# 0215Arthur/Pytorch_News_Recommender

Measured on AMD Instinct MI355X. Metric: users/sec (train step) NRMS MIND-small hist=50 cand=5, higher is better.
Workload: dtype f16 (MFMA inputs and saved activations; fp32 accumulate, softmax, loss, master weights and Adam); 1 GPU; configs[1] shapes: NRMS(nrms_v0) train step, 512 users/GPU, hist=50, cand=5, title_len=30, d=300, h=10, q=200, V=45800, dropout=0.2, Adam(lr=1e-3); users_per_gpu=512, global_batch=512, parallelism=dp1, precision=fp16, resident_batches=32

## Files before the change

### pytorch_news_recommender_amd/csrc/embed.hip

```cpp
#include "gemm.h"

#include <algorithm>

namespace nrms {

__global__ __launch_bounds__(256) void gather_dropout_kernel(unsigned total4, unsigned d4, const int64_t* ids,
                                                             const float* table, Dropout drop, float* x) {
    const unsigned stride = gridDim.x * blockDim.x;
    for (unsigned i = blockIdx.x * blockDim.x + threadIdx.x; i < total4; i += stride) {
        const unsigned m = i / d4, c4 = i - m * d4;
        const long id = ids[m];
        f32x4 v = *reinterpret_cast<const f32x4*>(table + id * (long)(4 * d4) + 4 * c4);
        if (drop.thresh != 0u) v *= dropout_scale4(drop.seed, 0u, (uint64_t)i, drop.thresh, drop.inv_keep);
        reinterpret_cast<f32x4*>(x)[i] = v;
    }
}

__global__ __launch_bounds__(256) void gather_dropout_compact_kernel(unsigned d4, const int64_t* ids, const int* live,
                                                                     const int* n_live, const float* table, Dropout drop,
                                                                     float* x) {
    const unsigned total4 = (unsigned)(*n_live) * d4;
    const unsigned stride = gridDim.x * blockDim.x;
    for (unsigned i = blockIdx.x * blockDim.x + threadIdx.x; i < total4; i += stride) {
        const unsigned r = i / d4, c4 = i - r * d4;
        const long t = live[r];
        f32x4 v = *reinterpret_cast<const f32x4*>(table + ids[t] * (long)(4 * d4) + 4 * c4);
        if (drop.thresh != 0u) v *= dropout_scale4(drop.seed, 0u, (uint64_t)(t * d4 + c4), drop.thresh, drop.inv_keep);
        reinterpret_cast<f32x4*>(x)[i] = v;
    }
}

int launch_gather_dropout_compact(long M, int d, const int64_t* ids, const int* live, const int* n_live,
                                  const float* table, const Dropout& drop, float* x, hipStream_t stream) {
    if (M <= 0) return NRMS_OK;
    if (M * (d / 4) >= (1L << 32)) { set_error("gather: %ld float4 elements overflow the 32-bit index", M * (d / 4)); return NRMS_EINVAL; }
    int blocks = cdiv(M * (d / 4), 256);
    if (blocks > 256 * 16) blocks = 256 * 16;
    TimingScope ts("gather_dropout", stream);
    hipLaunchKernelGGL(gather_dropout_compact_kernel, dim3(blocks), dim3(256), 0, stream, (unsigned)(d / 4), ids, live,
                       n_live, table, drop, x);
    return check_launch("gather_dropout");
}

template <bool SKIP_ALL_PAD, int FILL_SLICES>
__global__ __launch_bounds__(256) void fill_pad_rows_kernel_t(long n_seq, int S, int n4, const int64_t* ids, const float* row,
                                                              float* out) {
    const int lane = threadIdx.x & 63;
    const long wave = (long)blockIdx.x * 4 + (threadIdx.x >> 6), n_waves = (long)gridDim.x * 4;
    f32x4 b[FILL_SLICES];
#pragma unroll
    for (int i = 0; i < FILL_SLICES; ++i)
        b[i] = (lane + 64 * i < n4) ? reinterpret_cast<const f32x4*>(row)[lane + 64 * i] : f32x4{0.f, 0.f, 0.f, 0.f};
    for (long q = wave; q < n_seq; q += n_waves) {
        const bool is_pad = lane < S && ids[q * S + lane] == 0;
        unsigned long long m = __ballot(is_pad);
        if (SKIP_ALL_PAD && __popcll(m) == S) continue;
        while (m != 0ull) {
            const int r = __builtin_ctzll(m);
            m &= m - 1ull;
            f32x4* o = reinterpret_cast<f32x4*>(out) + (q * S + r) * n4;
#pragma unroll
            for (int i = 0; i < FILL_SLICES; ++i)
                if (lane + 64 * i < n4) o[lane + 64 * i] = b[i];
        }
    }
}

int launch_fill_pad_rows(long n_seq, int S, int n, const int64_t* ids, const float* row, float* out, bool skip_all_pad,
                         hipStream_t stream) {
    if (n_seq <= 0) return NRMS_OK;
    if ((n & 3) != 0 || n > 256 * 12 || S > 64) { set_error("fill_pad_rows: n=%d S=%d unsupported", n, S); return NRMS_EINVAL; }
    int blocks = cdiv(n_seq, 4);
    if (blocks > 256 * 32) blocks = 256 * 32;
    TimingScope ts("fill_pad_rows", stream);
    const bool wide = n > 256 * 6;
    auto go = [&](auto kernel) { hipLaunchKernelGGL(kernel, dim3(blocks), dim3(256), 0, stream, n_seq, S, n / 4, ids, row, out); };
    if (skip_all_pad) { if (wide) go(fill_pad_rows_kernel_t<true, 12>); else go(fill_pad_rows_kernel_t<true, 6>); }
    else { if (wide) go(fill_pad_rows_kernel_t<false, 12>); else go(fill_pad_rows_kernel_t<false, 6>); }
    return check_launch("fill_pad_rows");
}

constexpr int CP_BLOCK = 1024;
__global__ __launch_bounds__(256) void compact_count_kernel(long M, const int64_t* ids, int* counts) {
    __shared__ int wsum[4];
    const long m0 = (long)blockIdx.x * CP_BLOCK;
    int c = 0;
#pragma unroll
    for (int p = 0; p < 4; ++p) {
        const long m = m0 + p * 256 + threadIdx.x;
        c += (m < M && ids[m] != 0) ? 1 : 0;
    }
    c = (int)wave_sum((float)c);
    if ((threadIdx.x & 63) == 0) wsum[threadIdx.x >> 6] = c;
    __syncthreads();
    if (threadIdx.x == 0) counts[blockIdx.x] = wsum[0] + wsum[1] + wsum[2] + wsum[3];
}

__global__ __launch_bounds__(1024) void compact_scan_kernel(int n_blocks, int* counts, int* n_live) {
    __shared__ int buf[1024];
    __shared__ int carry;
    if (threadIdx.x == 0) carry = 0;
    __syncthreads();
    for (int base = 0; base < n_blocks; base += 1024) {
        const int i = base + threadIdx.x;
        const int v = i < n_blocks ? counts[i] : 0;
        buf[threadIdx.x] = v;
        __syncthreads();
        for (int off = 1; off < 1024; off <<= 1) {
            const int t = threadIdx.x >= off ? buf[threadIdx.x - off] : 0;
            __syncthreads();
            buf[threadIdx.x] += t;
            __syncthreads();
        }
        if (i < n_blocks) counts[i] = carry + buf[threadIdx.x] - v;
        __syncthreads();
        if (threadIdx.x == 1023) carry += buf[1023];
        __syncthreads();
    }
    if (threadIdx.x == 0) *n_live = carry;
}

__global__ __launch_bounds__(256) void compact_write_kernel(long M, const int64_t* ids, const int* offsets, int* live,
                                                            int* pos) {
    __shared__ int wave_cnt[4][4];
    const int lane = threadIdx.x & 63, wave = threadIdx.x >> 6;
    const long m0 = (long)blockIdx.x * CP_BLOCK;
    bool flag[4];
    int pre[4];
#pragma unroll
    for (int p = 0; p < 4; ++p) {
        const long m = m0 + p * 256 + threadIdx.x;
        flag[p] = m < M && ids[m] != 0;
        const unsigned long long b = __ballot(flag[p]);
        pre[p] = __popcll(b & ((1ull << lane) - 1ull));
        if (lane == 0) wave_cnt[p][wave] = __popcll(b);
    }
    __syncthreads();
    if (threadIdx.x == 0) {
        int tot = 0;
        for (int p = 0; p < 4; ++p)
            for (int w = 0; w < 4; ++w) { const int c = wave_cnt[p][w]; wave_cnt[p][w] = tot; tot += c; }
    }
    __syncthreads();
    const int base = offsets[blockIdx.x];
#pragma unroll
    for (int p = 0; p < 4; ++p) {
        const long m = m0 + p * 256 + threadIdx.x;
        const int r = base + wave_cnt[p][wave] + pre[p];
        if (flag[p]) live[r] = (int)m;
        if (pos != nullptr && m < M) pos[m] = flag[p] ? r : -1;
    }
}

size_t compact_scratch_ints(long M) { return (size_t)cdiv(M, CP_BLOCK) + 64; }

int launch_compact_live_rows(long M, const int64_t* ids, int* live, int* pos, int* n_live, int* scratch,
                             hipStream_t stream) {
    if (M <= 0) return NRMS_OK;
    const int nb = cdiv(M, CP_BLOCK);
    TimingScope ts("compact_rows", stream);
    hipLaunchKernelGGL(compact_count_kernel, dim3(nb), dim3(256), 0, stream, M, ids, scratch);
    hipLaunchKernelGGL(compact_scan_kernel, dim3(1), dim3(1024), 0, stream, nb, scratch, n_live);
    hipLaunchKernelGGL(compact_write_kernel, dim3(nb), dim3(256), 0, stream, M, ids, scratch, live, pos);
    return check_launch("compact_live_rows");
}

template <typename IDX>
__global__ __launch_bounds__(256) void scatter_dropout_compact_kernel(unsigned d, const int64_t* ids, const int* live,
                                                                      const int* n_live, const float* dx, Dropout drop,
                                                                      float* dtable) {
    const IDX total = (IDX)(*n_live) * d;
    const IDX stride = (IDX)gridDim.x * blockDim.x;
    for (IDX i = (IDX)blockIdx.x * blockDim.x + threadIdx.x; i < total; i += stride) {
        const IDX r = i / d;
        const unsigned c = (unsigned)(i - r * d);
        const long t = live[r];
        const long id = ids[t];
        float v = dx[i];
        if (drop.thresh != 0u) v *= dropout_scale1(drop.seed, 0u, (uint64_t)(t * d + c), drop.thresh, drop.inv_keep);
        atomicAdd(dtable + id * (long)d + c, v);
    }
}

__global__ __launch_bounds__(256) void scatter_dense_rows_kernel(unsigned d, const int64_t* ids, const int* live,
                                                                 const int* n_live, const float* dx, Dropout drop, float* dtable) {
    const unsigned long total = (unsigned long)(*n_live) * d;
    const unsigned long stride = (unsigned long)gridDim.x * blockDim.x;
    for (unsigned long i = (unsigned long)blockIdx.x * blockDim.x + threadIdx.x; i < total; i += stride) {
        const unsigned long r = i / d;
        const unsigned c = (unsigned)(i - r * d);
        const long t = live[r];
        float v = dx[t * (long)d + c];
        if (drop.thresh != 0u) v *= dropout_scale1(drop.seed, 0u, (uint64_t)(t * d + c), drop.thresh, drop.inv_keep);
        atomicAdd(dtable + ids[t] * (long)d + c, v);
    }
}

int launch_scatter_dense_rows(long M, int d, const int64_t* ids, const int* live, const int* n_live, const float* dx,
                              const Dropout& drop, float* dtable, hipStream_t stream) {
    if (M <= 0) return NRMS_OK;
    int blocks = cdiv(M * d, 256);
    if (blocks > 256 * 16) blocks = 256 * 16;
    TimingScope ts("scatter_dropout", stream);
    hipLaunchKernelGGL(scatter_dense_rows_kernel, dim3(blocks), dim3(256), 0, stream, (unsigned)d, ids, live, n_live, dx, drop, dtable);
    return check_launch("scatter_dense_rows");
}

int launch_scatter_dropout_compact(long M, int d, const int64_t* ids, const int* live, const int* n_live, const float* dx,
                                   const Dropout& drop, float* dtable, hipStream_t stream) {
    if (M <= 0) return NRMS_OK;
    int blocks = cdiv(M * d, 256);
    if (blocks > 256 * 16) blocks = 256 * 16;
    TimingScope ts("scatter_dropout", stream);
    if (M * d < (1L << 32))
        hipLaunchKernelGGL(scatter_dropout_compact_kernel<unsigned>, dim3(blocks), dim3(256), 0, stream, (unsigned)d, ids,
                           live, n_live, dx, drop, dtable);
    else
        hipLaunchKernelGGL(scatter_dropout_compact_kernel<unsigned long>, dim3(blocks), dim3(256), 0, stream, (unsigned)d, ids,
                           live, n_live, dx, drop, dtable);
    return check_launch("scatter_dropout");
}

__global__ __launch_bounds__(256) void tok_hist_kernel(const int64_t* ids, const int* live, const int* n_live, int* cnt) {
    const int n = *n_live;
    for (int r = blockIdx.x * blockDim.x + threadIdx.x; r < n; r += gridDim.x * blockDim.x)
        atomicAdd(cnt + ids[live[r]], 1);
}

__global__ __launch_bounds__(1024) void scan_local_kernel(int n, int* data, int* bsum) {
    __shared__ int buf[1024];
    const int i = blockIdx.x * 1024 + threadIdx.x;
    const int v = i < n ? data[i] : 0;
    buf[threadIdx.x] = v;
    __syncthreads();
    for (int off = 1; off < 1024; off <<= 1) {
        const int t = threadIdx.x >= off ? buf[threadIdx.x - off] : 0;
        __syncthreads();
        buf[threadIdx.x] += t;
        __syncthreads();
    }
    if (i < n) data[i] = buf[threadIdx.x] - v;
    if (threadIdx.x == 1023) bsum[blockIdx.x] = buf[1023];
}

__global__ __launch_bounds__(1024) void scan_add_kernel(int n, int n_blocks, int* data, const int* bsum, int* total) {
    __shared__ int base;
    if (threadIdx.x == 0) {
        int s = 0;
        for (int b = 0; b < (int)blockIdx.x; ++b) s += bsum[b];
        base = s;
        if (blockIdx.x == n_blocks - 1) *total = s + bsum[blockIdx.x];
    }
    __syncthreads();
    const int i = blockIdx.x * 1024 + threadIdx.x;
    if (i < n) data[i] += base;
}

__global__ __launch_bounds__(256) void tok_place_kernel(const int64_t* ids, const int* live, const int* n_live,
                                                        const int* offs, int* cursor, int* order) {
    const int n = *n_live;
    for (int r = blockIdx.x * blockDim.x + threadIdx.x; r < n; r += gridDim.x * blockDim.x) {
        const long id = ids[live[r]];
        order[offs[id] + atomicAdd(cursor + id, 1)] = r;
    }
}

typedef _Float16 sg_h4 __attribute__((ext_vector_type(4)));
template <bool H16, int SL>
__device__ __forceinline__ void bucket_sum(f32x4 (&s)[SL], int lane, int d4, int beg, int end, const int* live, const int* order,
                                           const void* dxv, int ldx, const Dropout& drop) {
    const float* dx = reinterpret_cast<const float*>(dxv);
    const _Float16* dx16 = reinterpret_cast<const _Float16*>(dxv);
    auto add_row = [&](int r) {
        const long t = live[r];
#pragma unroll
        for (int j = 0; j < SL; ++j) {
            const int c4 = lane + 64 * j;
            if (c4 < d4) {
                f32x4 g;
                if (H16) {
                    const sg_h4 gh = *reinterpret_cast<const sg_h4*>(dx16 + (long)r * ldx + 4 * c4);
#pragma unroll
                    for (int e = 0; e < 4; ++e) g[e] = (float)gh[e];
                } else {
                    g = *reinterpret_cast<const f32x4*>(dx + ((long)r * d4 + c4) * 4);
                }
                if (drop.thresh != 0u) g *= dropout_scale4(drop.seed, 0u, (uint64_t)(t * d4 + c4), drop.thresh, drop.inv_keep);
                s[j] += g;
            }
        }
    };
    constexpr int NONE = 0x7fffffff;
    for (int k0 = beg; k0 < end; k0 += 256) {
        const int n = min(256, end - k0);
        int m0 = lane < n ? order[k0 + lane] : NONE, m1 = lane + 64 < n ? order[k0 + 64 + lane] : NONE;
        int m2 = lane + 128 < n ? order[k0 + 128 + lane] : NONE, m3 = lane + 192 < n ? order[k0 + 192 + lane] : NONE;
        for (int i = 0; i < n; ++i) {
            int m = min(min(m0, m1), min(m2, m3));
#pragma unroll
            for (int o = 32; o > 0; o >>= 1) m = min(m, __shfl_xor(m, o, 64));
            add_row(m);
            m0 = m0 == m ? NONE : m0;
            m1 = m1 == m ? NONE : m1;
            m2 = m2 == m ? NONE : m2;
            m3 = m3 == m ? NONE : m3;
        }
    }
}

template <bool H16, int SL = 2>
__global__ __launch_bounds__(256) void scatter_grouped_kernel(int V, int d4, const int* live, const int* offs,
                                                              const int* total, const int* order, const void* dxv, int ldx,
                                                              const float* sc, Dropout drop, float* dtable) {
    const int lane = threadIdx.x & 63;
    const int v = blockIdx.x * 4 + (threadIdx.x >> 6);
    if (v >= V || v == 0) return;
    const int beg = offs[v], end = v + 1 < V ? offs[v + 1] : *total;
    if (beg == end) return;
    f32x4 s[SL];
#pragma unroll
    for (int j = 0; j < SL; ++j) s[j] = f32x4{0.f, 0.f, 0.f, 0.f};
    bucket_sum<H16, SL>(s, lane, d4, beg, end, live, order, dxv, ldx, drop);
#pragma unroll
    for (int j = 0; j < SL; ++j) {
        const int c4 = lane + 64 * j;
        if (c4 < d4) *reinterpret_cast<f32x4*>(dtable + ((long)v * d4 + c4) * 4) += H16 ? s[j] * sc[1] : s[j];
    }
}

template <bool H16, int SL, bool GUARD>
__global__ __launch_bounds__(256) void scatter_grouped_adam_kernel(int V, int d4, const int* live, const int* offs,
                                                                   const int* total, const int* order, const void* dxv, int ldx,
                                                                   const float* sc, Dropout drop, float* dtable, TableAdam a) {
    const int lane = threadIdx.x & 63;
    const int v = blockIdx.x * 4 + (threadIdx.x >> 6);
    if (v >= V) return;
    f32x4 s[SL];
#pragma unroll
    for (int j = 0; j < SL; ++j) s[j] = f32x4{0.f, 0.f, 0.f, 0.f};
    if (v != 0) {
        const int beg = offs[v], end = v + 1 < V ? offs[v + 1] : *total;
        bucket_sum<H16, SL>(s, lane, d4, beg, end, live, order, dxv, ldx, drop);
    }
    const long row4 = (long)v * d4;
    int bad = 0;
#pragma unroll
    for (int j = 0; j < SL; ++j) {
        const int c4 = lane + 64 * j;
        if (c4 < d4) {
            f32x4 g = f32x4{0.f, 0.f, 0.f, 0.f};
            g += H16 ? s[j] * sc[1] : s[j];
            f32x4 pv = reinterpret_cast<const f32x4*>(a.p)[row4 + c4];
            f32x4 mv = reinterpret_cast<const f32x4*>(a.m)[row4 + c4];
            f32x4 vv = reinterpret_cast<const f32x4*>(a.v)[row4 + c4];
            reinterpret_cast<f32x4*>(dtable)[row4 + c4] = g;
            const f32x4 gv = g * a.gscale;
#pragma unroll
            for (int e = 0; e < 4; ++e) {
                const bool skip = GUARD && (__float_as_uint(gv[e]) & 0x7F800000u) == 0x7F800000u;
                float pe = pv[e], me = mv[e], ve = vv[e];
                adam_update(pe, me, ve, gv[e], a.c.step_size, a.c.b1, a.c.b2, a.c.omb1, a.c.omb2, a.c.inv_sqrt_bc2, a.c.eps);
                pv[e] = skip ? pv[e] : pe; mv[e] = skip ? mv[e] : me; vv[e] = skip ? vv[e] : ve;
                bad += skip ? 1 : 0;
            }
            reinterpret_cast<f32x4*>(a.p)[row4 + c4] = pv;
            reinterpret_cast<f32x4*>(a.m)[row4 + c4] = mv;
            reinterpret_cast<f32x4*>(a.v)[row4 + c4] = vv;
        }
    }
    if (GUARD) {
#pragma unroll
        for (int o = 32; o > 0; o >>= 1) bad += __shfl_xor(bad, o, 64);
        if (bad != 0 && lane == 0) atomicAdd(a.n_bad, bad);
    }
}

static size_t scan_blocks(int V) { return (size_t)cdiv(V, 1024); }
size_t scatter_grouped_scratch_ints(long M, int V) { return (size_t)2 * (V + 64) + std::max((size_t)M, scan_blocks(V)) + 64; }

int launch_scatter_prepare(long M, int V, const int64_t* ids, const int* live, const int* n_live, int* scratch, hipStream_t stream) {
    if (M <= 0) return NRMS_OK;
    int* cnt = scratch;
    int* cursor = cnt + V + 64;
    int* total = cursor + V;
    int* order = cursor + V + 64;
    if (hipMemsetAsync(cnt, 0, (size_t)(2 * (V + 64)) * sizeof(int), stream) != hipSuccess) {
        set_error("scatter_grouped: memset failed");
        return NRMS_ELAUNCH;
    }
    int blocks = cdiv(M, 256);
    if (blocks > 2048) blocks = 2048;
    TimingScope ts("scatter_prepare", stream);
    hipLaunchKernelGGL(tok_hist_kernel, dim3(blocks), dim3(256), 0, stream, ids, live, n_live, cnt);
    {
        const int nb = (int)scan_blocks(V);
        int* bsum = order;
        hipLaunchKernelGGL(scan_local_kernel, dim3(nb), dim3(1024), 0, stream, V, cnt, bsum);
        hipLaunchKernelGGL(scan_add_kernel, dim3(nb), dim3(1024), 0, stream, V, nb, cnt, bsum, total);
    }
    hipLaunchKernelGGL(tok_place_kernel, dim3(blocks), dim3(256), 0, stream, ids, live, n_live, cnt, cursor, order);
    return check_launch("scatter_prepare");
}

int launch_scatter_grouped(long M, int V, int d, const int64_t* ids, const int* live, const int* n_live, const void* dx,
                           const Dropout& drop, float* dtable, int* scratch, hipStream_t stream, bool dx_fp16, int ldx,
                           const float* sc, bool prepared) {
    if (M <= 0) return NRMS_OK;
    if ((d & 3) != 0 || d > 1024 || (dx_fp16 && d > 512)) { set_error("scatter_grouped: d=%d unsupported", d); return NRMS_EINVAL; }
    if (!prepared) {
        const int rc = launch_scatter_prepare(M, V, ids, live, n_live, scratch, stream);
        if (rc) return rc;
    }
    int* cnt = scratch;
    int* cursor = cnt + V + 64;
    int* total = cursor + V;
    int* order = cursor + V + 64;
    TimingScope ts("scatter_dropout", stream);
    if (dx_fp16)
        hipLaunchKernelGGL(scatter_grouped_kernel<true>, dim3(cdiv(V, 4)), dim3(256), 0, stream, V, d / 4, live, cnt, total, order, dx,
                           ldx, sc, drop, dtable);
    else if (d <= 512)
        hipLaunchKernelGGL(scatter_grouped_kernel<false>, dim3(cdiv(V, 4)), dim3(256), 0, stream, V, d / 4, live, cnt, total, order, dx,
                           d, nullptr, drop, dtable);
    else
        hipLaunchKernelGGL((scatter_grouped_kernel<false, 4>), dim3(cdiv(V, 4)), dim3(256), 0, stream, V, d / 4, live, cnt, total, order,
                           dx, d, nullptr, drop, dtable);
    return check_launch("scatter_grouped");
}

int launch_scatter_grouped_adam(long M, int V, int d, const int64_t* ids, const int* live, const int* n_live, const void* dx,
                                const Dropout& drop, float* dtable, int* scratch, hipStream_t stream, bool dx_fp16, int ldx,
                                const float* sc, bool prepared, const TableAdam& a) {
    if (M <= 0 || V <= 0) { set_error("scatter_grouped_adam: nothing to scatter (the caller runs the plain Adam step)"); return NRMS_EINVAL; }
    if ((d & 3) != 0 || d > 1024 || (dx_fp16 && d > 512)) { set_error("scatter_grouped_adam: d=%d unsupported", d); return NRMS_EINVAL; }
    if (!prepared) {
        const int rc = launch_scatter_prepare(M, V, ids, live, n_live, scratch, stream);
        if (rc) return rc;
    }
    int* cnt = scratch;
    int* cursor = cnt + V + 64;
    int* total = cursor + V;
    int* order = cursor + V + 64;
    const bool guard = a.n_bad != nullptr;
    TimingScope ts("adam", stream);
    auto go = [&](auto kernel, int ld, const float* scp) {
        hipLaunchKernelGGL(kernel, dim3(cdiv(V, 4)), dim3(256), 0, stream, V, d / 4, live, cnt, total, order, dx, ld, scp, drop, dtable, a);
    };
    if (dx_fp16) { if (guard) go(scatter_grouped_adam_kernel<true, 2, true>, ldx, sc); else go(scatter_grouped_adam_kernel<true, 2, false>, ldx, sc); }
    else if (d <= 512) { if (guard) go(scatter_grouped_adam_kernel<false, 2, true>, d, nullptr); else go(scatter_grouped_adam_kernel<false, 2, false>, d, nullptr); }
    else { if (guard) go(scatter_grouped_adam_kernel<false, 4, true>, d, nullptr); else go(scatter_grouped_adam_kernel<false, 4, false>, d, nullptr); }
    return check_launch("scatter_grouped_adam");
}

template <class SRC>
__global__ __launch_bounds__(256) void sanitize_ids_kernel(long n, const SRC* src, int64_t* dst, long vocab, int* n_bad) {
    int bad = 0;
    for (long i = (long)blockIdx.x * blockDim.x + threadIdx.x; i < n; i += (long)gridDim.x * blockDim.x) {
        const int64_t v = (int64_t)src[i];
        const bool ok = v >= 0 && v < vocab;
        bad += ok ? 0 : 1;
        dst[i] = ok ? v : 0;
    }
    const unsigned long long m = __ballot(bad != 0);
    if (m != 0ull) {
        bad = (int)wave_sum((float)bad);
        if ((threadIdx.x & 63) == 0) atomicAdd(n_bad, bad);
    }
}

int launch_sanitize_ids(long n, const void* src, bool src_is_int32, int64_t* dst, int vocab, int* n_bad, hipStream_t stream) {
    if (n <= 0) return NRMS_OK;
    int blocks = cdiv(n, 256 * 4);
    if (blocks > 256 * 8) blocks = 256 * 8;
    TimingScope ts("sanitize_ids", stream);
    if (src_is_int32)
        hipLaunchKernelGGL(sanitize_ids_kernel<int32_t>, dim3(blocks), dim3(256), 0, stream, n, (const int32_t*)src, dst, (long)vocab, n_bad);
    else
        hipLaunchKernelGGL(sanitize_ids_kernel<int64_t>, dim3(blocks), dim3(256), 0, stream, n, (const int64_t*)src, dst, (long)vocab, n_bad);
    return check_launch("sanitize_ids");
}

__global__ __launch_bounds__(256) void dedup_insert_kernel(long n, int L, const int64_t* ids, int* table, unsigned mask,
                                                           int* inverse, int* rep_rows, int* n_unique) {
    const int lane = threadIdx.x & 63;
    for (long t = (long)blockIdx.x * blockDim.x + threadIdx.x; t < n; t += (long)gridDim.x * blockDim.x) {
        const int64_t* row = ids + t * L;
        uint64_t h = 0x9E3779B97F4A7C15ull ^ (uint64_t)L;
        int64_t any = 0;
        for (int i = 0; i < L; ++i) {
            const int64_t w = row[i];
            any |= w;
            uint64_t k = (uint64_t)w * 0xFF51AFD7ED558CCDull;
            k ^= k >> 32;
            h = (h ^ k) * 0xC4CEB9FE1A85EC53ull;
            h ^= h >> 29;
        }
        h ^= h >> 33; h *= 0xFF51AFD7ED558CCDull; h ^= h >> 33;
        const bool pad = any == 0;
        const unsigned long long pads = __ballot(pad);
        const int leader = pads != 0 ? __ffsll((long long)pads) - 1 : 0;
        int result = 0;
        if (!pad || lane == leader) {
            unsigned slot = (unsigned)h & mask;
            for (;;) {
                int cur = __hip_atomic_load(table + slot, __ATOMIC_RELAXED, __HIP_MEMORY_SCOPE_AGENT);
                if (cur < 0) {
                    cur = atomicCAS(table + slot, -1, (int)t);
                    if (cur < 0) {
                        const int u = atomicAdd(n_unique, 1);
                        rep_rows[u] = (int)t;
                        result = u;
                        break;
                    }
                }
                const int64_t* other = ids + (long)cur * L;
                bool same = true;
                for (int i = 0; i < L; ++i) same = same && other[i] == row[i];
                if (same) { result = -cur - 1; break; }
                slot = (slot + 1) & mask;
            }
        }
        const int lead = __shfl(result, leader);
        inverse[t] = (pad && lane != leader) ? lead : result;
    }
}

__global__ __launch_bounds__(256) void dedup_resolve_kernel(long n, int* inverse) {
    for (long t = (long)blockIdx.x * blockDim.x + threadIdx.x; t < n; t += (long)gridDim.x * blockDim.x) {
        const int v = inverse[t];
        if (v < 0) inverse[t] = inverse[-v - 1];
    }
}

int launch_title_dedup(long n, int L, const int64_t* ids, int* table, long table_size, int* inverse, int* rep_rows,
                       int* n_unique, hipStream_t stream) {
    if (hipMemsetAsync(n_unique, 0, sizeof(int), stream) != hipSuccess) { set_error("title_dedup: memset failed"); return NRMS_ELAUNCH; }
    if (n <= 0) return NRMS_OK;
    if (hipMemsetAsync(table, 0xFF, (size_t)table_size * sizeof(int), stream) != hipSuccess) {
        set_error("title_dedup: memset failed");
        return NRMS_ELAUNCH;
    }
    int blocks = cdiv(n, 256);
    if (blocks > 256 * 16) blocks = 256 * 16;
    TimingScope ts("title_dedup", stream);
    hipLaunchKernelGGL(dedup_insert_kernel, dim3(blocks), dim3(256), 0, stream, n, L, ids, table, (unsigned)(table_size - 1),
                       inverse, rep_rows, n_unique);
    hipLaunchKernelGGL(dedup_resolve_kernel, dim3(blocks), dim3(256), 0, stream, n, inverse);
    return check_launch("title_dedup");
}

int launch_gather_dropout(long M, int d, const int64_t* ids, const float* table, const Dropout& drop, float* x,
                          hipStream_t stream) {
    if (M <= 0) return NRMS_OK;
    const long total4 = M * (d / 4);
    if (total4 >= (1L << 32)) { set_error("gather: %ld float4 elements overflow the 32-bit index", total4); return NRMS_EINVAL; }
    int blocks = cdiv(total4, 256);
    if (blocks > 256 * 16) blocks = 256 * 16;
    TimingScope ts("gather_dropout", stream);
    hipLaunchKernelGGL(gather_dropout_kernel, dim3(blocks), dim3(256), 0, stream, (unsigned)total4, (unsigned)(d / 4),
                       ids, table, drop, x);
    return check_launch("gather_dropout");
}

}
```

Before: 180,500 users/s.

## Rank-sort bucket rows once and prefetch rows ahead in grouped embedding scatter

Replaces the per-row wave-wide min-reduction in the grouped embedding-gradient scatter with a one-time rank computation. Each bucket's row indices are ordered by readlane comparisons and a permute, then walked with a software-pipelined loop that loads upcoming rows a fixed lookahead ahead of the accumulation. This is meant to remove the serial shuffle reduction per row and to hide gather latency. The change uses more registers for the prefetched rows and adds code complexity. The old min-select path stays available behind an environment variable and remains the only path for SL=4.

Result: no change. 182,000 users/s, median of 6 (+0.8%).

```diff
diff --git a/pytorch_news_recommender_amd/csrc/embed.hip b/pytorch_news_recommender_amd/csrc/embed.hip
--- a/pytorch_news_recommender_amd/csrc/embed.hip
+++ b/pytorch_news_recommender_amd/csrc/embed.hip
@@ -1,6 +1,8 @@
 #include "gemm.h"
 
 #include <algorithm>
+#include <stdlib.h>
+#include <type_traits>
 
 namespace nrms {
 
@@ -266,11 +268,12 @@
 }
 
 typedef _Float16 sg_h4 __attribute__((ext_vector_type(4)));
-template <bool H16, int SL>
+template <bool H16, int SL, bool MINSEL, int LA>
 __device__ __forceinline__ void bucket_sum(f32x4 (&s)[SL], int lane, int d4, int beg, int end, const int* live, const int* order,
                                            const void* dxv, int ldx, const Dropout& drop) {
     const float* dx = reinterpret_cast<const float*>(dxv);
     const _Float16* dx16 = reinterpret_cast<const _Float16*>(dxv);
+    typedef typename std::conditional<H16, sg_h4, f32x4>::type row_t;
     auto add_row = [&](int r) {
         const long t = live[r];
 #pragma unroll
@@ -290,9 +293,31 @@
             }
         }
     };
+    auto load_row_all = [&](row_t (&q)[SL], int r) {
+#pragma unroll
+        for (int j = 0; j < SL; ++j) {
+            const int c4 = min(lane + 64 * j, d4 - 1);
+            if constexpr (H16) q[j] = *reinterpret_cast<const sg_h4*>(dx16 + (long)r * ldx + 4 * c4);
+            else q[j] = *reinterpret_cast<const f32x4*>(dx + ((long)r * d4 + c4) * 4);
+        }
+    };
+    auto add_row_all = [&](const row_t (&q)[SL], long t) {
+#pragma unroll
+        for (int j = 0; j < SL; ++j) {
+            const int c4 = lane + 64 * j;
+            f32x4 g;
+            if constexpr (H16) {
+#pragma unroll
+                for (int e = 0; e < 4; ++e) g[e] = (float)q[j][e];
+            } else {
+                g = q[j];
+            }
+            if (drop.thresh != 0u) g *= dropout_scale4(drop.seed, 0u, (uint64_t)(t * d4 + c4), drop.thresh, drop.inv_keep);
+            s[j] += g;
+        }
+    };
     constexpr int NONE = 0x7fffffff;
-    for (int k0 = beg; k0 < end; k0 += 256) {
-        const int n = min(256, end - k0);
+    auto minsel_chunk = [&](int k0, int n) {
         int m0 = lane < n ? order[k0 + lane] : NONE, m1 = lane + 64 < n ? order[k0 + 64 + lane] : NONE;
         int m2 = lane + 128 < n ? order[k0 + 128 + lane] : NONE, m3 = lane + 192 < n ? order[k0 + 192 + lane] : NONE;
         for (int i = 0; i < n; ++i) {
@@ -305,10 +330,87 @@
             m2 = m2 == m ? NONE : m2;
             m3 = m3 == m ? NONE : m3;
         }
-    }
-}
-
-template <bool H16, int SL = 2>
+    };
+    if constexpr (MINSEL || SL == 4) {
+        for (int k0 = beg; k0 < end; k0 += 256) minsel_chunk(k0, min(256, end - k0));
+        return;
+    }
+    constexpr int LA_SHORT = LA, LA_LONG = 0;
+    auto walk = [&](auto la, int n, auto entry) {
+        constexpr int A = decltype(la)::value, R = A + 1;
+        row_t q[R][SL];
+        int r, t;
+        if (n <= A) {
+#pragma unroll
+            for (int a = 0; a < A; ++a)
+                if (a < n) { entry(a, r, t); load_row_all(q[a], r); }
+#pragma unroll
+            for (int a = 0; a < A; ++a)
+                if (a < n) { entry(a, r, t); add_row_all(q[a], (long)t); }
+            return;
+        }
+#pragma unroll
+        for (int a = 0; a < A; ++a) { entry(a, r, t); load_row_all(q[a], r); }
+        for (int i = 0;;) {
+#pragma unroll
+            for (int u = 0; u < R; ++u) {
+                entry(min(i + A, n - 1), r, t);
+                load_row_all(q[(u + A) % R], r);
+                entry(i, r, t);
+                add_row_all(q[u], (long)t);
+                if (++i == n) return;
+            }
+        }
+    };
+    const int kbeg = __builtin_amdgcn_readfirstlane(beg), kend = __builtin_amdgcn_readfirstlane(end);
+    for (int k0 = kbeg; k0 < kend; k0 += 256) {
+        const int n = min(256, kend - k0);
+        if (n <= 64) {
+            int m0 = lane < n ? order[k0 + lane] : NONE;
+            int t0 = lane < n ? live[m0] : 0;
+            if (n > 1) {
+                int rk = 0;
+                for (int j = 0; j < n; ++j) rk += __builtin_amdgcn_readlane(m0, j) < m0 ? 1 : 0;
+                rk = lane < n ? rk : lane;
+                m0 = __builtin_amdgcn_ds_permute(rk << 2, m0);
+                t0 = __builtin_amdgcn_ds_permute(rk << 2, t0);
+            }
+            walk(std::integral_constant<int, LA_SHORT>{}, n, [&](int i, int& r, int& t) {
+                r = __builtin_amdgcn_readlane(m0, i);
+                t = __builtin_amdgcn_readlane(t0, i);
+            });
+        } else {
+            int m[4], t4[4], rk[4];
+#pragma unroll
+            for (int q = 0; q < 4; ++q) {
+                m[q] = lane + 64 * q < n ? order[k0 + 64 * q + lane] : NONE;
+                rk[q] = 0;
+            }
+#pragma unroll
+            for (int q = 0; q < 4; ++q) t4[q] = lane + 64 * q < n ? live[m[q]] : 0;
+#pragma unroll
+            for (int q = 0; q < 4; ++q) {
+                const int cnt = min(64, n - 64 * q);
+                for (int j = 0; j < cnt; ++j) {
+                    const int key = __builtin_amdgcn_readlane(m[q], j);
+#pragma unroll
+                    for (int p = 0; p < 4; ++p) rk[p] += key < m[p] ? 1 : 0;
+                }
+            }
+            walk(std::integral_constant<int, LA_LONG>{}, n, [&](int i, int& r, int& t) {
+                const bool h0 = rk[0] == i, h1 = rk[1] == i, h2 = rk[2] == i, h3 = rk[3] == i;
+                const int mk = h0 ? m[0] : h1 ? m[1] : h2 ? m[2] : h3 ? m[3] : 0;
+                const int tk = h0 ? t4[0] : h1 ? t4[1] : h2 ? t4[2] : h3 ? t4[3] : 0;
+                const unsigned long long hit = __ballot(h0 || h1 || h2 || h3);
+                const int src = hit != 0ull ? __builtin_ctzll(hit) : 0;
+                r = __builtin_amdgcn_readlane(mk, src);
+                t = __builtin_amdgcn_readlane(tk, src);
+            });
+        }
+    }
+}
+
+template <bool H16, int SL, bool MINSEL>
 __global__ __launch_bounds__(256) void scatter_grouped_kernel(int V, int d4, const int* live, const int* offs,
                                                               const int* total, const int* order, const void* dxv, int ldx,
                                                               const float* sc, Dropout drop, float* dtable) {
@@ -320,7 +422,7 @@
     f32x4 s[SL];
 #pragma unroll
     for (int j = 0; j < SL; ++j) s[j] = f32x4{0.f, 0.f, 0.f, 0.f};
-    bucket_sum<H16, SL>(s, lane, d4, beg, end, live, order, dxv, ldx, drop);
+    bucket_sum<H16, SL, MINSEL, H16 ? 2 : 0>(s, lane, d4, beg, end, live, order, dxv, ldx, drop);
 #pragma unroll
     for (int j = 0; j < SL; ++j) {
         const int c4 = lane + 64 * j;
@@ -328,7 +430,7 @@
     }
 }
 
-template <bool H16, int SL, bool GUARD>
+template <bool H16, int SL, bool GUARD, bool MINSEL>
 __global__ __launch_bounds__(256) void scatter_grouped_adam_kernel(int V, int d4, const int* live, const int* offs,
                                                                    const int* total, const int* order, const void* dxv, int ldx,
                                                                    const float* sc, Dropout drop, float* dtable, TableAdam a) {
@@ -340,7 +442,7 @@
     for (int j = 0; j < SL; ++j) s[j] = f32x4{0.f, 0.f, 0.f, 0.f};
     if (v != 0) {
         const int beg = offs[v], end = v + 1 < V ? offs[v + 1] : *total;
-        bucket_sum<H16, SL>(s, lane, d4, beg, end, live, order, dxv, ldx, drop);
+        bucket_sum<H16, SL, MINSEL, H16 ? 2 : 1>(s, lane, d4, beg, end, live, order, dxv, ldx, drop);
     }
     const long row4 = (long)v * d4;
     int bad = 0;
@@ -402,6 +504,11 @@
     return check_launch("scatter_prepare");
 }
 
+static bool walk_minsel() {
+    const char* e = getenv("NRMS_SCATTER_WALK_MINSEL");
+    return e != nullptr && atoi(e) != 0;
+}
+
 int launch_scatter_grouped(long M, int V, int d, const int64_t* ids, const int* live, const int* n_live, const void* dx,
                            const Dropout& drop, float* dtable, int* scratch, hipStream_t stream, bool dx_fp16, int ldx,
                            const float* sc, bool prepared) {
@@ -415,16 +522,14 @@
     int* cursor = cnt + V + 64;
     int* total = cursor + V;
     int* order = cursor + V + 64;
+    const bool minsel = walk_minsel();
     TimingScope ts("scatter_dropout", stream);
-    if (dx_fp16)
-        hipLaunchKernelGGL(scatter_grouped_kernel<true>, dim3(cdiv(V, 4)), dim3(256), 0, stream, V, d / 4, live, cnt, total, order, dx,
-                           ldx, sc, drop, dtable);
-    else if (d <= 512)
-        hipLaunchKernelGGL(scatter_grouped_kernel<false>, dim3(cdiv(V, 4)), dim3(256), 0, stream, V, d / 4, live, cnt, total, order, dx,
-                           d, nullptr, drop, dtable);
-    else
-        hipLaunchKernelGGL((scatter_grouped_kernel<false, 4>), dim3(cdiv(V, 4)), dim3(256), 0, stream, V, d / 4, live, cnt, total, order,
-                           dx, d, nullptr, drop, dtable);
+    auto go = [&](auto kernel, int ld, const float* scp) {
+        hipLaunchKernelGGL(kernel, dim3(cdiv(V, 4)), dim3(256), 0, stream, V, d / 4, live, cnt, total, order, dx, ld, scp, drop, dtable);
+    };
+    if (dx_fp16) { if (minsel) go(scatter_grouped_kernel<true, 2, true>, ldx, sc); else go(scatter_grouped_kernel<true, 2, false>, ldx, sc); }
+    else if (d <= 512) { if (minsel) go(scatter_grouped_kernel<false, 2, true>, d, nullptr); else go(scatter_grouped_kernel<false, 2, false>, d, nullptr); }
+    else { if (minsel) go(scatter_grouped_kernel<false, 4, true>, d, nullptr); else go(scatter_grouped_kernel<false, 4, false>, d, nullptr); }
     return check_launch("scatter_grouped");
 }
 
@@ -441,14 +546,20 @@
     int* cursor = cnt + V + 64;
     int* total = cursor + V;
     int* order = cursor + V + 64;
-    const bool guard = a.n_bad != nullptr;
+    const bool guard = a.n_bad != nullptr, minsel = walk_minsel();
     TimingScope ts("adam", stream);
     auto go = [&](auto kernel, int ld, const float* scp) {
         hipLaunchKernelGGL(kernel, dim3(cdiv(V, 4)), dim3(256), 0, stream, V, d / 4, live, cnt, total, order, dx, ld, scp, drop, dtable, a);
     };
-    if (dx_fp16) { if (guard) go(scatter_grouped_adam_kernel<true, 2, true>, ldx, sc); else go(scatter_grouped_adam_kernel<true, 2, false>, ldx, sc); }
-    else if (d <= 512) { if (guard) go(scatter_grouped_adam_kernel<false, 2, true>, d, nullptr); else go(scatter_grouped_adam_kernel<false, 2, false>, d, nullptr); }
-    else { if (guard) go(scatter_grouped_adam_kernel<false, 4, true>, d, nullptr); else go(scatter_grouped_adam_kernel<false, 4, false>, d, nullptr); }
+    auto pick = [&](auto h16, auto sl, int ld, const float* scp) {
+        constexpr bool H = decltype(h16)::value;
+        constexpr int S = decltype(sl)::value;
+        if (minsel) { if (guard) go(scatter_grouped_adam_kernel<H, S, true, true>, ld, scp); else go(scatter_grouped_adam_kernel<H, S, false, true>, ld, scp); }
+        else { if (guard) go(scatter_grouped_adam_kernel<H, S, true, false>, ld, scp); else go(scatter_grouped_adam_kernel<H, S, false, false>, ld, scp); }
+    };
+    if (dx_fp16) pick(std::true_type{}, std::integral_constant<int, 2>{}, ldx, sc);
+    else if (d <= 512) pick(std::false_type{}, std::integral_constant<int, 2>{}, d, nullptr);
+    else pick(std::false_type{}, std::integral_constant<int, 4>{}, d, nullptr);
     return check_launch("scatter_grouped_adam");
 }
 
```
